# Berkeley-Speech-Group/sylber

Measured on AMD Instinct MI355X. Metric: audio-sec/s encoded (sylber_base, 16 kHz, batched 10 s clips), higher is better.
Workload: dtype bf16

## Files before the change

### include/sylber_hip.h

```cpp
#ifndef SYLBER_HIP_H
#define SYLBER_HIP_H

#include <stdint.h>

#ifdef __cplusplus
extern "C" {
#endif

#define SYLBER_MAX_LAYERS 12
#define SYLBER_HIDDEN 768
#define SYLBER_CONV_DIM 512

typedef struct sylber_ctx* sylber_t;

enum { SYLBER_BF16 = 0, SYLBER_FP32 = 1, SYLBER_FP8 = 2, SYLBER_FP16 = 3, SYLBER_MIXED16 = 4, SYLBER_SPLIT16 = 5 };

typedef struct {
    const float* q_w; const float* q_b;
    const float* k_w; const float* k_b;
    const float* v_w; const float* v_b;
    const float* o_w; const float* o_b;
    const float* ln1_w; const float* ln1_b;
    const float* ff1_w; const float* ff1_b;
    const float* ff2_w; const float* ff2_b;
// ... 78 lines not shown
int sylber_mlp_create(const SylberMlpWeights* w, int device, sylber_mlp_t* out);
void sylber_mlp_destroy(sylber_mlp_t m);
int64_t sylber_condition_workspace_floats(sylber_mlp_t m, int32_t B, int32_t S);
int sylber_condition(sylber_mlp_t m, const float* hidden_dev, const int64_t* seg_dev, const int32_t* nseg_dev, const float* feat_dev,
                     int32_t B, int32_t T, int32_t S, float norm_thr, float* avg_hidden_dev, float* cond_dev, float* workspace_dev,
                     void* stream);

int64_t sylber_condition_units_workspace_floats(sylber_mlp_t m, int32_t B, int32_t S);
int sylber_condition_units(sylber_mlp_t m, const float* c1_dev, int32_t K1, const float* c2_dev, int32_t K2, const int32_t* units_dev,
                           const int32_t* spans_dev, const int32_t* nunits_dev, const int32_t* frames_dev, int32_t B, int32_t T, int32_t S,
                           float* cond_dev, float* workspace_dev, void* stream);
int64_t sylber_condition_packed_workspace_floats(sylber_mlp_t m, int32_t B, int32_t S);
int sylber_condition_packed(sylber_mlp_t m, const float* hidden_dev, const int32_t* offsets_host, const int32_t* frames_host, int32_t B,
                            const int64_t* seg_dev, const int32_t* nseg_dev, const float* feat_dev, int32_t K, int32_t S, float norm_thr,
                            float* avg_hidden_dev, float* cond_dev, float* workspace_dev, void* stream);
int sylber_condition_units_packed(sylber_mlp_t m, const float* c1_dev, int32_t K1, const float* c2_dev, int32_t K2, const int32_t* units_dev,
                                  const int32_t* spans_dev, const int32_t* nunits_dev, const int32_t* frames_host, int32_t B, int32_t S,
                                  float* cond_dev, float* workspace_dev, void* stream);
int sylber_expand_units(const float* feats_dev, const int32_t* durations_dev, int32_t B, int32_t S, int32_t D, int32_t T, float* out_dev,
                        int32_t* workspace_dev, void* stream);

enum { SYLBER_OPT_GEMM_TILE = 1, SYLBER_OPT_ATTN_QUERIES_PER_WAVE = 2, SYLBER_OPT_GEMM_PERSISTENT = 3, SYLBER_OPT_FUSE_OUTPROJ_LN = 4,
       SYLBER_OPT_CONV0_VALU = 5, SYLBER_OPT_RESLN_PREFETCH = 6, SYLBER_OPT_FP8_ATTENTION = 7, SYLBER_OPT_GEMM_TAIL = 8, SYLBER_OPT_SEGMENT = 9, SYLBER_OPT_FP16_AUDIT = 10, SYLBER_OPT_GEMM_H192 = 11, SYLBER_OPT_GEMM_MODEL = 12, SYLBER_OPT_GEMM_MFMA16 = 13,
       SYLBER_OPT_PER_UTTERANCE = 14 };
int sylber_set_option(sylber_t h, int32_t key, int32_t value);
int sylber_get_fp16_audit(sylber_t h, const char** names, uint32_t* saturated, float* max_abs, int32_t cap);

int sylber_condition_features(sylber_mlp_t m, const float* features_dev, int32_t rows, float* cond_dev, float* workspace_dev,
                              void* stream);

int sylber_set_stop_stage(sylber_t h, int32_t stage);
int sylber_set_profiling(sylber_t h, int32_t enable);
int sylber_get_profile(sylber_t h, const char** names, float* ms, int32_t cap);
int sylber_set_graph_mode(sylber_t h, int32_t enable);
int64_t sylber_workspace_bytes(sylber_t h);

#define SYLBER_CFM_DEPTH 8
typedef struct {
    const float *attn_gamma_w, *attn_gamma_b, *attn_beta_w, *attn_beta_b;
    const float *q_gamma, *k_gamma;
    const float *qkv_w, *out_w;
    const float *ff_gamma_w, *ff_gamma_b, *ff_beta_w, *ff_beta_b;
    const float *ff1_w, *ff1_b, *ff2_w, *ff2_b;
} SylberCfmLayer;
typedef struct {
    const float *proj_in_w, *proj_in_b;
    const float *time_freq, *time_w, *time_b;
// ... 41 lines not shown
```

### include/sylber_hip_dev.h

```cpp
#ifndef SYLBER_HIP_DEV_H
#define SYLBER_HIP_DEV_H
#include <stdint.h>
#include "sylber_hip.h"
#ifdef __cplusplus
extern "C" {
#endif
int sylber_debug_gemm_bench(int32_t M, int32_t N, int32_t K, int32_t ldx, int32_t epi, int32_t act, int32_t cfg,
                            int32_t iters, float* ms_out);
int sylber_debug_gemm_pick(int32_t M, int32_t N, int32_t K, int32_t epi, int32_t act, int32_t fmt, int32_t model, int32_t kpat);
int sylber_debug_gemm_trace(int32_t M, int32_t N, int32_t K, int32_t ldx, int32_t epi, int32_t act, unsigned long long* out20,
                            float* ms_out);
int sylber_debug_poison_workspace(sylber_t h, int32_t byte);
int sylber_debug_attention_bench(int32_t B, int32_t T, int32_t precision, int32_t iters, float* ms_out);
#ifdef __cplusplus
}
#endif
#endif
```

### sylber_amd/_lib.py

```python
from __future__ import annotations

import ctypes
import os
from ctypes import POINTER, c_char_p, c_float, c_int, c_int32, c_int64, c_void_p

_HERE = os.path.dirname(os.path.abspath(__file__))
LIB_PATH = os.path.join(_HERE, "libsylber_hip.so")
_DEV_LIB = False
MAX_LAYERS = 12

c_float_p = POINTER(c_float)


class SylberLayerWeights(ctypes.Structure):
    _fields_ = [(n, c_float_p) for n in (
        "q_w", "q_b", "k_w", "k_b", "v_w", "v_b", "o_w", "o_b", "ln1_w", "ln1_b",
        "ff1_w", "ff1_b", "ff2_w", "ff2_b", "ln2_w", "ln2_b")]


class SylberMlpHidden(ctypes.Structure):
    _fields_ = [(n, c_float_p) for n in ("lin_w", "lin_b", "ff1_w", "ff1_b", "ff2_w", "ff2_b", "ln_w", "ln_b")]


class SylberMlpWeights(ctypes.Structure):
# ... 90 lines not shown
    "sylber_packed_layout": (c_int, [POINTER(c_int32), c_int32, POINTER(c_int32), POINTER(c_int32)]),
    "sylber_forward_packed": (c_int, [c_void_p, c_void_p, POINTER(c_int32), c_int32, c_void_p, c_void_p]),
    "sylber_packed_gather": (c_int, [c_void_p, POINTER(c_int32), c_int32, c_void_p, c_void_p]),
    "sylber_segment_packed": (c_int, [c_void_p, c_void_p, POINTER(c_int32), c_int32, c_float, c_float, c_void_p, c_void_p, c_void_p,
                                      c_void_p]),
    "sylber_cfm_packed_layout": (c_int, [POINTER(c_int32), c_int32, POINTER(c_int32)]),
    "sylber_cfm_workspace_bytes_packed": (c_int64, [c_void_p, POINTER(c_int32), c_int32]),
    "sylber_cfm_sample_packed": (c_int, [c_void_p, c_void_p, POINTER(c_int32), c_int32, c_int32, c_void_p, c_float, c_void_p, c_void_p,
                                         c_void_p]),
    "sylber_condition_packed_workspace_floats": (c_int64, [c_void_p, c_int32, c_int32]),
    "sylber_condition_packed": (c_int, [c_void_p, c_void_p, POINTER(c_int32), POINTER(c_int32), c_int32, c_void_p, c_void_p, c_void_p,
                                        c_int32, c_int32, c_float, c_void_p, c_void_p, c_void_p, c_void_p]),
    "sylber_condition_units_packed": (c_int, [c_void_p, c_void_p, c_int32, c_void_p, c_int32, c_void_p, c_void_p, c_void_p,
                                              POINTER(c_int32), c_int32, c_int32, c_void_p, c_void_p, c_void_p]),
    "sylber_op_attention": (c_int, [c_void_p, c_void_p, c_void_p, c_void_p, c_void_p, c_int32, c_int32, c_int32,
                                    c_int32, c_void_p]),
}
DEV_EXPORTS = {
    "sylber_debug_gemm_bench": (c_int, [c_int32] * 8 + [POINTER(c_float)]),
    "sylber_debug_gemm_pick": (c_int, [c_int32] * 8),
    "sylber_debug_gemm_trace": (c_int, [c_int32] * 6 + [POINTER(ctypes.c_uint64), POINTER(c_float)]),
    "sylber_debug_attention_bench": (c_int, [c_int32] * 4 + [POINTER(c_float)]),
    "sylber_debug_poison_workspace": (c_int, [c_void_p, c_int32]),
}
OPT_GEMM_TILE, OPT_ATTN_QUERIES_PER_WAVE, OPT_GEMM_PERSISTENT = 1, 2, 3
OPT_CONV0_VALU = 5
OPT_FP8_ATTENTION, OPT_SEGMENT, OPT_PER_UTTERANCE = 7, 9, 14

_LIB = None


class SylberHipError(RuntimeError):
    pass


def load() -> ctypes.CDLL:
    global _LIB
    if _LIB is None:
        if not os.path.exists(LIB_PATH):
            raise SylberHipError(
                "libsylber_hip.so is not built (%s). Run `python -c 'import __graft_entry__ as g; g.build()'` "
                "or `python sylber_amd/build.py`; there is no CPU fallback on the product path." % LIB_PATH)
        lib = ctypes.CDLL(LIB_PATH)
        for name, (res, args) in list(EXPORTS.items()) + list(DEV_EXPORTS.items()):
            if _DEV_LIB and not hasattr(lib, name):
                continue
            fn = getattr(lib, name)
            fn.restype = res
            fn.argtypes = args
        _LIB = lib
# ... 14 lines not shown
```

### sylber_amd/csrc/api.hip

```cpp
#include <stdio.h>
#include <stdlib.h>
#include <string.h>

#include <string>
#include <vector>

#include "../../include/sylber_hip.h"
#include "../../include/sylber_hip_dev.h"
#include "kernels.h"

static thread_local char g_err[512] = "";
void syl_set_error(const char* what, const char* detail) { snprintf(g_err, sizeof(g_err), "%s: %s", what, detail); }
extern "C" const char* sylber_last_error(void) { return g_err; }

struct DeviceGuard {
    int prev = -1; bool ok = true;
    explicit DeviceGuard(int dev) {
        if (hipGetDevice(&prev) != hipSuccess) prev = -1;
        if (prev != dev) ok = hipSetDevice(dev) == hipSuccess;
    }
    ~DeviceGuard() { int cur = -1; if (prev >= 0 && hipGetDevice(&cur) == hipSuccess && cur != prev) (void)hipSetDevice(prev); }
};
#define GUARD_DEVICE(dev)                                                                             \
    DeviceGuard _dg(dev);                                                                             \
// ... 36 lines not shown
    return 0;
}

struct LayerDev {
    bf16_t *wqkv, *wo, *w1, *w2;
    uint8_t *w1q = nullptr, *w1s = nullptr, *w2q = nullptr, *w2s = nullptr;
    uint8_t *wqkvq = nullptr, *wqkvs = nullptr;
    uint8_t *woq = nullptr, *wos = nullptr;
    float *bqkv, *bo, *b1, *b2, *ln1w, *ln1b, *ln2w, *ln2b;
};

struct ProfEntry { std::string name; hipEvent_t e0, e1; };
struct GraphEntry { int B, Lmax, stop_stage; const void* in; void* out; hipGraphExec_t exec; unsigned long long stamp; };

struct sylber_ctx {
    int device = 0, precision = 0, num_layers = 9;
    int fmt = FMT_BF16;
    int fmt_conv = FMT_BF16;
    char* wbase = nullptr; size_t wbytes = 0;
    char* f8base = nullptr; size_t f8bytes = 0;
    float *conv0_w, *gn_w, *gn_b, *fp_ln_w, *fp_ln_b, *fp_b, *pos_b, *enc_ln_w, *enc_ln_b;
    bf16_t* conv_w[7];
    bf16_t *fp_w, *pos_w;
    LayerDev L[SYLBER_MAX_LAYERS];
    float* conv_w32[7]; float *fp_w32, *pos_w32;
    struct { float *wqkv, *wo, *w1, *w2; } L32[SYLBER_MAX_LAYERS];
    char* ws = nullptr; size_t ws_bytes = 0;
    int ws_B = 0, ws_Lmax = 0;
    float* seg_scratch = nullptr; size_t seg_scratch_floats = 0;
    int stop_stage = 0;
    int opt_gemm_cfg = 0, opt_attn_qw = 0, opt_gemm_persist = 0;
    int opt_fuse_ln = 0;
    int opt_conv0_valu = 0;
    int opt_audit16 = 0;
    unsigned* audit_dev = nullptr;
    int opt_segment = 0;
    int opt_gemm_model = 0;
    int opt_gemm_mfma16 = 0;
    int opt_gemm_h192 = 0;
    int opt_gemm_tail = 0;
    int opt_attn8 = 0;
    int opt_resln_pre = 0;
    int opt_per_utt = 0;
    bool graph_mode = false;
    std::vector<GraphEntry> graphs; unsigned long long graph_clock = 0;
    int profiling = 0;
    std::vector<ProfEntry> prof;
    std::vector<hipEvent_t> ev_pool;
    std::vector<std::string> prof_names; std::vector<float> prof_ms;
};

struct Packer {
    std::vector<char> host;
    size_t add(size_t bytes) { size_t off = (host.size() + 255) & ~(size_t)255; host.resize(off + bytes); return off; }
    size_t add_f32(const float* src, size_t n) { size_t o = add(n * 4); memcpy(host.data() + o, src, n * 4); return o; }
    int fmt = FMT_BF16;
    size_t add_bf16(const float* src, size_t n) {
        if (fmt == FMT_SPLIT) {
            size_t o = add(n * 4);
            bf16_t* d = (bf16_t*)(host.data() + o);
            for (size_t i = 0; i < n; ++i) { d[i] = f2h_host(src[i]); d[n + i] = f2h_host(src[i] - h2f_host(d[i])); }
            return o;
        }
        size_t o = add(n * 2);
        bf16_t* d = (bf16_t*)(host.data() + o);
        if (fmt == FMT_F16) for (size_t i = 0; i < n; ++i) d[i] = f2h_host(src[i]);
// ... 35 lines not shown
    }
    P.fmt = c->fmt;
    size_t o_fplw = P.add_f32(w->fp_ln_w, 512), o_fplb = P.add_f32(w->fp_ln_b, 512);
    size_t o_fpw = f32 ? P.add_f32(w->fp_w, 768 * 512) : P.add_bf16(w->fp_w, 768 * 512), o_fpb = P.add_f32(w->fp_b, 768);
    size_t o_posw;
    {
        std::vector<float> tmp((size_t)16 * 128 * 64 * 56, 0.f);
        for (int g = 0; g < 16; ++g)
            for (int n = 0; n < 48; ++n)
                for (int cc = 0; cc < 48; ++cc)
                    for (int t = 0; t < 128; ++t)
                        tmp[(((size_t)g * 128 + t) * 64 + n) * 56 + cc] = w->pos_w[(((size_t)g * 48 + n) * 48 + cc) * 128 + t];
        if (!f32) o_posw = P.add_bf16(tmp.data(), tmp.size());
        else {
            std::vector<float> t32((size_t)16 * 128 * 64 * 52, 0.f);
            for (int g = 0; g < 16; ++g)
                for (int n = 0; n < 48; ++n)
                    for (int cc = 0; cc < 48; ++cc)
                        for (int t = 0; t < 128; ++t)
                            t32[(((size_t)g * 128 + t) * 64 + n) * 52 + cc] = w->pos_w[(((size_t)g * 48 + n) * 48 + cc) * 128 + t];
            o_posw = P.add_f32(t32.data(), t32.size());
        }
    }
    size_t o_posb = P.add_f32(w->pos_b, 768);
    size_t o_elw = P.add_f32(w->enc_ln_w, 768), o_elb = P.add_f32(w->enc_ln_b, 768);
    struct LOff { size_t wqkv, bqkv, wo, bo, l1w, l1b, w1, b1, w2, b2, l2w, l2b; } lo[SYLBER_MAX_LAYERS];
    for (int l = 0; l < w->num_layers; ++l) {
        const SylberLayerWeights& lw = w->layers[l];
        std::vector<float> qkv((size_t)2304 * 768), bq(2304);
        memcpy(qkv.data(), lw.q_w, 768 * 768 * 4);
        memcpy(qkv.data() + 768 * 768, lw.k_w, 768 * 768 * 4);
        memcpy(qkv.data() + 2 * 768 * 768, lw.v_w, 768 * 768 * 4);
        memcpy(bq.data(), lw.q_b, 768 * 4); memcpy(bq.data() + 768, lw.k_b, 768 * 4); memcpy(bq.data() + 1536, lw.v_b, 768 * 4);
        lo[l].wqkv = f32 ? P.add_f32(qkv.data(), qkv.size()) : P.add_bf16(qkv.data(), qkv.size()); lo[l].bqkv = P.add_f32(bq.data(), 2304);
        lo[l].wo = f32 ? P.add_f32(lw.o_w, 768 * 768) : P.add_bf16(lw.o_w, 768 * 768); lo[l].bo = P.add_f32(lw.o_b, 768);
        lo[l].l1w = P.add_f32(lw.ln1_w, 768); lo[l].l1b = P.add_f32(lw.ln1_b, 768);
        lo[l].w1 = f32 ? P.add_f32(lw.ff1_w, (size_t)3072 * 768) : P.add_bf16(lw.ff1_w, (size_t)3072 * 768); lo[l].b1 = P.add_f32(lw.ff1_b, 3072);
        lo[l].w2 = f32 ? P.add_f32(lw.ff2_w, (size_t)768 * 3072) : P.add_bf16(lw.ff2_w, (size_t)768 * 3072); lo[l].b2 = P.add_f32(lw.ff2_b, 768);
        lo[l].l2w = P.add_f32(lw.ln2_w, 768); lo[l].l2b = P.add_f32(lw.ln2_b, 768);
    }
    c->wbytes = P.host.size();
    if (hipMalloc((void**)&c->wbase, c->wbytes) != hipSuccess) { delete c; syl_set_error("sylber_create", "hipMalloc(weights) failed"); return 1; }
    if (hipMemcpy(c->wbase, P.host.data(), c->wbytes, hipMemcpyHostToDevice) != hipSuccess) {
        hipFree(c->wbase); delete c; syl_set_error("sylber_create", "weight upload failed"); return 1;
    }
    char* b = c->wbase;
    c->conv0_w = (float*)(b + o_conv0); c->gn_w = (float*)(b + o_gnw); c->gn_b = (float*)(b + o_gnb);
    c->conv_w[0] = nullptr;
    for (int i = 1; i < 7; ++i) { c->conv_w[i] = (bf16_t*)(b + o_conv[i]); c->conv_w32[i] = (float*)(b + o_conv[i]); }
    c->fp_w32 = (float*)(b + o_fpw); c->pos_w32 = (float*)(b + o_posw);
    c->fp_ln_w = (float*)(b + o_fplw); c->fp_ln_b = (float*)(b + o_fplb);
    c->fp_w = (bf16_t*)(b + o_fpw); c->fp_b = (float*)(b + o_fpb);
    c->pos_w = (bf16_t*)(b + o_posw); c->pos_b = (float*)(b + o_posb);
    c->enc_ln_w = (float*)(b + o_elw); c->enc_ln_b = (float*)(b + o_elb);
    for (int l = 0; l < w->num_layers; ++l) {
        LayerDev& d = c->L[l];
        d.wqkv = (bf16_t*)(b + lo[l].wqkv); d.bqkv = (float*)(b + lo[l].bqkv);
        d.wo = (bf16_t*)(b + lo[l].wo); d.bo = (float*)(b + lo[l].bo);
        d.ln1w = (float*)(b + lo[l].l1w); d.ln1b = (float*)(b + lo[l].l1b);
        d.w1 = (bf16_t*)(b + lo[l].w1); d.b1 = (float*)(b + lo[l].b1);
        d.w2 = (bf16_t*)(b + lo[l].w2); d.b2 = (float*)(b + lo[l].b2);
        d.ln2w = (float*)(b + lo[l].l2w); d.ln2b = (float*)(b + lo[l].l2b);
        c->L32[l].wqkv = (float*)(b + lo[l].wqkv); c->L32[l].wo = (float*)(b + lo[l].wo);
        c->L32[l].w1 = (float*)(b + lo[l].w1); c->L32[l].w2 = (float*)(b + lo[l].w2);
    }
    if (precision == SYLBER_FP8) {
        const size_t per_layer = (size_t)3072 * 768 + (size_t)3072 * 24 + (size_t)768 * 3072 + (size_t)768 * 96 +
                                 (size_t)2304 * 768 + (size_t)2304 * 24 + (size_t)768 * 768 + (size_t)768 * 24;
        c->f8bytes = per_layer * w->num_layers;
        float* tmp = nullptr;
        if (hipMalloc((void**)&c->f8base, c->f8bytes) != hipSuccess || hipMalloc((void**)&tmp, (size_t)3072 * 768 * 4) != hipSuccess) {
            if (c->f8base) hipFree(c->f8base);
            hipFree(c->wbase); delete c; syl_set_error("sylber_create", "hipMalloc(fp8 weights) failed"); return 1;
        }
        int bad = 0;
        for (int l = 0; l < w->num_layers && !bad; ++l) {
// ... 48 lines not shown
        case SYLBER_OPT_GEMM_TILE: c->opt_gemm_cfg = value < 0 ? 0 : value + 1; break;
        case SYLBER_OPT_ATTN_QUERIES_PER_WAVE: c->opt_attn_qw = value == 32 ? 1 : (value == 64 ? 2 : 0); break;
        case SYLBER_OPT_GEMM_PERSISTENT: c->opt_gemm_persist = value; break;
        case SYLBER_OPT_FUSE_OUTPROJ_LN: c->opt_fuse_ln = value > 0 ? 1 : (value < 0 ? -1 : 0); break;
        case SYLBER_OPT_CONV0_VALU: c->opt_conv0_valu = value > 0 ? (value == 2 ? 2 : 1) : 0; break;
        case SYLBER_OPT_RESLN_PREFETCH: c->opt_resln_pre = value < 0 ? -1 : (value <= 3 ? value : 0); break;
        case SYLBER_OPT_FP8_ATTENTION: c->opt_attn8 = value < 0 ? -1 : (value > 0 ? 1 : 0); break;
        case SYLBER_OPT_FP16_AUDIT: {
            GUARD_DEVICE(c->device);
            c->opt_audit16 = value > 0 ? 1 : 0;
            if (c->opt_audit16) {
                if (!c->audit_dev) HIP_TRY(hipMalloc((void**)&c->audit_dev, AUDIT_STAGES * 2 * sizeof(unsigned)));
                HIP_TRY(hipDeviceSynchronize());
                HIP_TRY(hipMemset(c->audit_dev, 0, AUDIT_STAGES * 2 * sizeof(unsigned)));
            }
            break;
        }
        case SYLBER_OPT_SEGMENT: c->opt_segment = value < 0 ? -1 : 0; break;
        case SYLBER_OPT_GEMM_MODEL: c->opt_gemm_model = value == 5 ? 5 : (value == 2 ? 2 : (value == 6 ? 6 : 0)); break;
        case SYLBER_OPT_GEMM_H192: c->opt_gemm_h192 = value < 0 ? -1 : 0; break;
        case SYLBER_OPT_GEMM_MFMA16: c->opt_gemm_mfma16 = value < 0 ? -1 : 0; break;
        case SYLBER_OPT_GEMM_TAIL: c->opt_gemm_tail = value < 0 ? -1 : (value > 0 ? value + 1 : 0); break;
        case SYLBER_OPT_PER_UTTERANCE: c->opt_per_utt = value == 1 ? 1 : 0; break;
        default: syl_set_error("sylber_set_option", "unknown option key"); return 1;
    }
    if (c->graph_mode) { for (auto& g : c->graphs) if (g.exec) hipGraphExecDestroy(g.exec); c->graphs.clear(); }
    return 0;
}
extern "C" int sylber_set_profiling(sylber_t c, int32_t enable) {
    if (!c) return 1;
    const char* nm[1]; float ms[1];
    sylber_get_profile(c, nm, ms, 0);
    c->prof_names.clear(); c->prof_ms.clear();
    c->profiling = enable;
    return 0;
}
extern "C" int64_t sylber_workspace_bytes(sylber_t c) { return c ? (int64_t)(c->ws_bytes + c->seg_scratch_floats * 4 + c->wbytes + c->f8bytes) : 0; }

struct Plan {
    int B, Lmax, L[7], T, Tp, Tpv, R[7];
    size_t o_bufA, o_bufB, o_ln512, o_xf32, o_xpad, o_pre, o_stats, o_hbf16, o_q, o_k, o_vt, o_ctx, o_ffn, o_part, o_ss, o_valid,
        o_rows, o_pk, total;
    int nchunk;
    bool zero_all = false;
    long lo_bufA = 0, lo_bufB = 0, lo_ln512 = 0, lo_xpad = 0, lo_hbf = 0, lo_qk = 0, lo_vt = 0, lo_ctx = 0, lo_ffn = 0;
};
// ... 241 lines not shown
        bf16_t* t = src; src = dst; dst = t;
        const long tl = src_lo; src_lo = dst_lo; dst_lo = tl;
    }
    bf16_t* feats = src;
    const long feats_lo = src_lo;
    if (c->stop_stage == 1) {
        RUN("copy_out", launch_bf16_to_f32_rows(feats, 512, hidden_dev, B, p.Tp, p.T, 512, s, c->fmt_conv, feats_lo));
        return 0;
    }
    {
        LnArgs a = {};
        a.in = feats; a.in_bf16 = 1; a.ld_in = 512; a.gamma = c->fp_ln_w; a.beta = c->fp_ln_b;
        a.out_bf16 = ln512; a.ld_bf16 = 512; a.M = M; a.D = 512; a.fmt = c->fmt; a.fmt_in = c->fmt_conv;
        a.in_lo = feats_lo; a.out_lo = p.lo_ln512;
        RUN("ln512", launch_layernorm(a, s));
        GemmArgs g = {};
        g.X = ln512; g.ldx = 512; g.W = c->fp_w; g.M = M; g.N = 768; g.K = 512; g.bias = c->fp_b;
        g.out0 = xf32; g.ld0 = 768; g.out1 = xpad; g.Tp = p.Tp; g.T = p.T; g.valid = valid; g.xpad_rows = p.Tp + 128; g.fmt = c->fmt;
        g.x_lo = p.lo_ln512; g.w_lo = (long)768 * 512; g.out_lo = p.lo_xpad;
        RUN("gemm_proj", launch_gemm_bf16(EPI_PROJ, g, s));
        if (pk) RUN("zero_slot_tails", launch_zero_slot_tails(xf32, xpad, pk->slot, pk->frames, pk->nclip, pk->tail_max, s));
        if (aud_e && (audit16(c, AUD_LN512, ln512, M, 512, 512, s) || audit16(c, AUD_XPAD, xpad, (long)B * (p.Tp + 128), 768, 768, s))) return 1;
    }
    if (pk) RUN("posconv", launch_posconv_packed(xpad, c->pos_w, c->pos_b, xf32, pre, pk->nclip, pk->slot_max, pk->slot, pk->frames, s, c->fmt));
    else
    RUN("posconv", launch_posconv(xpad, c->pos_w, c->pos_b, xf32, pre, B, p.Tp, split ? 2 : 1, s, c->fmt, p.lo_xpad, (long)16 * 128 * 64 * 56));
    const bool f8 = c->precision == SYLBER_FP8;
    const long Mp = ((long)M + 255) & ~255L;
    uint8_t* h8 = (uint8_t*)hbf; uint8_t* h8s = h8 + (((size_t)M * 768 + 255) & ~(size_t)255);
    uint8_t* ctx8 = (uint8_t*)ctx; uint8_t* ctx8s = ctx8 + (((size_t)M * 768 + 255) & ~(size_t)255);
    uint8_t* ffn8 = (uint8_t*)ffn; uint8_t* ffn8s = ffn8 + (((size_t)M * 3072 + 255) & ~(size_t)255);
    auto run_ln = [&](const float* gam, const float* bet, bool last, bool to_fp8 = false) -> int {
        LnArgs a = {};
        a.in = pre; a.in_bf16 = 0; a.ld_in = 768; a.gamma = gam; a.beta = bet; a.M = M; a.D = 768; a.fmt = c->fmt; a.fmt_in = c->fmt;
        if (last) { a.out_f32 = hidden_dev; a.ld_f32 = 768; a.Tp = p.Tp; a.T = p.T; }
        else if (to_fp8) { a.out_fp8 = h8; a.ld_fp8 = 768; a.out_scale = h8s; a.scale_rows = Mp; a.out_stats = stats; }
        else { a.out_bf16 = hbf; a.ld_bf16 = 768; a.out_stats = stats; a.out_lo = p.lo_hbf; }
        if (launch_layernorm(a, s)) return 1;
        if (aud_e && !last && !to_fp8) return audit16(c, AUD_LN, hbf, M, 768, 768, s);
        return 0;
    };
    RUN("layernorm", run_ln(c->enc_ln_w, c->enc_ln_b, c->stop_stage == 2, f8));
    if (c->stop_stage == 2) return 0;
    const float* res_g = c->enc_ln_w; const float* res_b = c->enc_ln_b;
    for (int l = 0; l < c->num_layers; ++l) {
        const LayerDev& d = c->L[l];
        const bool last = (l == c->num_layers - 1) || (c->stop_stage == 3 + l);
        bool fused_ln1 = false;
        uint8_t* q8 = (uint8_t*)q; uint8_t* k8 = (uint8_t*)k; uint8_t* v8 = (uint8_t*)vt;
// ... 593 lines not shown
    if (qb.alloc(n * 2) || kb.alloc(n * 2 + 64 * 64 * 2) || vb.alloc((size_t)B * 768 * Tpv * 2) || cb.alloc(n * 2)) { syl_set_error("sylber_op_attention", "alloc"); return 1; }
    HIP_TRY(hipMemsetAsync(qb.p, 0, n * 2, s)); HIP_TRY(hipMemsetAsync(kb.p, 0, n * 2 + 64 * 64 * 2, s));
    HIP_TRY(hipMemsetAsync(vb.p, 0, (size_t)B * 768 * Tpv * 2, s)); HIP_TRY(hipMemsetAsync(cb.p, 0, n * 2, s));
    hipLaunchKernelGGL(pack_qkv_kernel, dim3(T, B), dim3(256), 0, s, q_dev, k_dev, v_dev, (bf16_t*)qb.p, (bf16_t*)kb.p, (bf16_t*)vb.p, T, Tp, Tpv);
    if (launch_attention((bf16_t*)qb.p, (bf16_t*)kb.p, (bf16_t*)vb.p, valid_dev, (bf16_t*)cb.p, B, T, Tp, Tpv, qw, s)) return 1;
    if (launch_bf16_to_f32_rows((bf16_t*)cb.p, 768, o_dev, B, Tp, T, 768, s)) return 1;
    HIP_TRY(hipStreamSynchronize(s));
    return 0;
}


__global__ void fill_random_bf16(bf16_t* p, size_t n, unsigned seed);
extern "C" int sylber_debug_poison_workspace(sylber_t c, int32_t byte) {
    if (!c) { syl_set_error("sylber_debug_poison_workspace", "null handle"); return 1; }
    GUARD_DEVICE(c->device);
    HIP_TRY(hipDeviceSynchronize());
    if (c->ws) HIP_TRY(hipMemset(c->ws, byte & 0xff, c->ws_bytes));
    if (c->seg_scratch) HIP_TRY(hipMemset(c->seg_scratch, byte & 0xff, c->seg_scratch_floats * 4));
    c->ws_B = 0; c->ws_Lmax = 0;
    if (c->graph_mode) { for (auto& g : c->graphs) if (g.exec) hipGraphExecDestroy(g.exec); c->graphs.clear(); }
    return 0;
}

extern "C" int sylber_debug_attention_bench(int32_t B, int32_t T, int32_t precision, int32_t iters, float* ms_out) {
    const int Tp = (T + 31) & ~31, Tpv = (Tp + 63) & ~63;
    const size_t n = (size_t)B * Tp * 768;
    TmpBuf qin;
    if (qin.alloc((size_t)B * T * 768 * 4 * 3)) { syl_set_error("sylber_debug_attention_bench", "alloc"); return 1; }
    float* q = (float*)qin.p; float* k = q + (size_t)B * T * 768; float* v = k + (size_t)B * T * 768;
    const bool zero_data = iters < 0;
    if (zero_data) { iters = -iters; HIP_TRY(hipMemset(qin.p, 0, (size_t)B * T * 768 * 4 * 3)); }
    else
    {
        TmpBuf tmp;
        if (tmp.alloc((size_t)B * T * 768 * 3 * 2)) { syl_set_error("sylber_debug_attention_bench", "alloc"); return 1; }
        hipLaunchKernelGGL(fill_random_bf16, dim3(2048), dim3(256), 0, 0, (bf16_t*)tmp.p, (size_t)B * T * 768 * 3, 7u);
        if (launch_bf16_to_f32_rows((bf16_t*)tmp.p, 768, q, 3 * B, T, T, 768, 0)) return 1;
        HIP_TRY(hipDeviceSynchronize());
    }
    hipEvent_t e0, e1;
    hipEventCreate(&e0); hipEventCreate(&e1);
    int rc = 0;
    if (precision == SYLBER_FP8) {
        AttnF8Bufs f;
        if (f.alloc(B, Tp, Tpv) || f.clear(B, Tp, Tpv, 0)) { syl_set_error("sylber_debug_attention_bench", "alloc"); return 1; }
        hipLaunchKernelGGL(pack_qk_f8_kernel, dim3(T, B), dim3(256), 0, 0, q, k, (uint8_t*)f.q8.p, (uint8_t*)f.qs.p, (uint8_t*)f.k8.p, (uint8_t*)f.ks.p, T, Tp);
// ... 183 lines not shown
```

### sylber_amd/csrc/kernels.h

```cpp
#pragma once
#include "common.h"

enum GemmAct { ACT_NONE = 0, ACT_GELU_FAST = 1, ACT_GELU_ERF = 2, ACT_GELU_ERF7 = 3 };
enum GemmEpi {
    EPI_BF16 = 0,
    EPI_F32 = 1,
    EPI_F32_RES = 2,
    EPI_QK = 3,
    EPI_PROJ = 4,
    EPI_MXFP8 = 7,
    EPI_QK8 = 8,
    EPI_F32_RESLN = 6,
};

struct GemmArgs {
    const bf16_t* X; long ldx;
    const bf16_t* W;
    int M, N, K;
    int M_store;
    const float* bias;
    int act;
    void* out0; long ld0;
    void* out1; void* out2;
    const float* res; long ldres;
// ... 47 lines not shown
enum GemmActF32 { ACTF_NONE = 0, ACTF_GELU_ERF = 1, ACTF_RELU = 2 };
struct GemmArgsF32 {
    const float* X; long ldx;
    const float* W;
    int M, N, K;
    const float* bias; int act;
    float* out0; long ld0;
    const float* res; long ldres;
    int Tp, T; const int* valid;
    float* xpad; int xpad_rows;
    int tiled;
};
int launch_gemm_f32(const GemmArgsF32& a, hipStream_t s);

int launch_conv0_stats(const float* wav, int B, int Lmax, int L0, double* partials, int nchunk, hipStream_t s, const int* rows = nullptr,
                       const int* slot = nullptr);
int launch_conv0_finalize(const double* partials, int nchunk, const float* w0, const float* gn_w, const float* gn_b,
                          int B, int L0, float* scale_shift, hipStream_t s, const int* rows = nullptr);
int launch_conv0_gn_gelu(const float* wav, int B, int Lmax, int L0, int R0, const float* w0,
                         const float* scale_shift, void* out, int out_f32, hipStream_t s, int fmt = 0, long out_lo = 0, int valu16 = 0);
int launch_conv0_packed(const float* wav, int B, int total_samples, int slot_max, const int* rows, const int* slot, const float* w0,
                        const float* scale_shift, bf16_t* out, int fmt, hipStream_t s);
int launch_zero_slot_tails(float* x, bf16_t* xpad, const int* slot, const int* frames, int B, int tail_max, hipStream_t s);
int launch_posconv_packed(const bf16_t* xpad, const bf16_t* wpk, const float* bias, const float* x_f32, float* out, int B, int slot_max,
                          const int* slot, const int* frames, hipStream_t s, int fmt);
int launch_attention_packed(const bf16_t* q, const bf16_t* k, const bf16_t* vt, const int* pk, int nclip, int total_qb, bf16_t* ctx,
                            int Ptot, hipStream_t s, int fmt);

struct LnArgs {
    const void* in; int in_bf16; long ld_in;
    int fmt;
    int fmt_in;
    const float* res; long ld_res;
    const float* gamma; const float* beta;
    float* out_f32; long ld_f32;
    bf16_t* out_bf16; long ld_bf16;
    uint8_t* out_fp8; long ld_fp8;
    uint8_t* out_scale; long scale_rows;
    float* out_stats;
    int M, D;
    int Tp, T;
    long in_lo, out_lo;
};
int launch_layernorm(const LnArgs& a, hipStream_t s);

int launch_attention(const bf16_t* q, const bf16_t* k, const bf16_t* vt, const int* valid, bf16_t* ctx, int B, int T,
                     int Tp, int Tpv, int qw, hipStream_t s, int fmt = 0, long lo_qk = 0, long lo_vt = 0, long lo_ctx = 0);
int launch_attention_f8(const uint8_t* q8, const uint8_t* qs, const uint8_t* k8, const uint8_t* ks, const uint8_t* v8, const uint8_t* vs,
                        const int* valid, void* ctx, uint8_t* ctx_scale, long scale_rows, int B, int T, int Tp, int Tpv, hipStream_t s);
int launch_attention_f8out(const bf16_t* q, const bf16_t* k, const bf16_t* vt, const int* valid, uint8_t* ctx8, uint8_t* ctx_scale,
                           long scale_rows, int B, int T, int Tp, int Tpv, int qw, hipStream_t s);
int launch_attention_f32(const float* q, const float* k, const float* v, const int* valid, float* ctx, int B, int T,
                         int Tp, hipStream_t s);

int launch_posconv(const bf16_t* xpad, const bf16_t* wpk, const float* bias, const float* x_f32, float* out, int B,
                   int Tp, int act, hipStream_t s, int fmt = 0, long x_lo = 0, long w_lo = 0);
int launch_posconv_f32(const float* xpad, const float* w, const float* bias, const float* x_f32, float* out, int B,
                       int Tp, hipStream_t s);

int launch_segment(const float* hidden, int B, int T, int D, float norm_thr, float merge_thr, int64_t* seg, int* nseg,
                   float* feat, float* scratch, hipStream_t s, int mode = 0, const int* frames = nullptr, const int* row0 = nullptr);
size_t segment_scratch_floats(int B, int T, int D);

int launch_upload_ints(int* dst, const int32_t* vals_host, int n, int add, hipStream_t s);
int launch_f32_to_bf16(const float* in, bf16_t* out, size_t n, hipStream_t s);
int launch_f32_to_split16(const float* in, bf16_t* out, long lo_off, size_t n, hipStream_t s);
int launch_bf16_to_f32_rows(const bf16_t* in, long ld_in, float* out, int B, int Tp, int T, int D, hipStream_t s, int fmt = 0, long in_lo = 0);
```

### sylber_amd/csrc/posconv.hip

```cpp
#include "kernels.h"

#define PC_BM 256
#define PC_XROW 112
#define PC_XWIN (384 * PC_XROW)
#define PC_SLAB (64 * 112)
#define PC_TAPS_PER_STEP 2
#define PC_STEP (PC_TAPS_PER_STEP * PC_SLAB)
#define PC_LDS (PC_XWIN + 2 * PC_STEP)

typedef __attribute__((address_space(3))) void* lds_vptr;
typedef const __attribute__((address_space(1))) void* glb_vptr;
__device__ __forceinline__ void glds16p(__amdgpu_buffer_rsrc_t rs, int voff, int soff, void* l) {
    __builtin_amdgcn_raw_ptr_buffer_load_lds(rs, (lds_vptr)l, 16, voff, soff, 0, 0);
}

template <int ACT, int FMT>
__global__ __launch_bounds__(512, 4) void posconv_bf16_kernel(const bf16_t* __restrict__ xpad, const bf16_t* __restrict__ wpk,
                                                              const float* __restrict__ bias, const float* __restrict__ x_f32,
                                                              float* __restrict__ out, int Tp, long x_lo, long w_lo,
                                                              const int* __restrict__ slot, const int* __restrict__ frames) {
    extern __shared__ __attribute__((aligned(256))) char smem[];
    char* xwin = smem;
    char* wring = smem + PC_XWIN;
    const int tid = threadIdx.x, wave = tid >> 6, lane = tid & 63;
// ... 71 lines not shown
    }
    const int t = t0 + wave * 32 + ql;
    if (t < Tpb) {
        const size_t m = slot ? (size_t)s0 + t : (size_t)b * Tp + t;
#pragma unroll
        for (int nf = 0; nf < 2; ++nf)
#pragma unroll
            for (int gg = 0; gg < 4; ++gg) {
                const int nl = 32 * nf + 8 * gg + 4 * h;
                if (nl >= SYL_POSC) continue;
                const int n = g * SYL_POSC + nl;
                const float4 bb = *(const float4*)(bias + n);
                const float4 rr = *(const float4*)(x_f32 + m * SYL_HIDDEN + n);
                float v0 = acc[nf][4 * gg + 0] + bb.x, v1 = acc[nf][4 * gg + 1] + bb.y;
                float v2 = acc[nf][4 * gg + 2] + bb.z, v3 = acc[nf][4 * gg + 3] + bb.w;
                if constexpr (ACT == 2 && FMT == FMT_SPLIT) { v0 = gelu_erf7(v0); v1 = gelu_erf7(v1); v2 = gelu_erf7(v2); v3 = gelu_erf7(v3); }
                else if constexpr (ACT == 2) { v0 = gelu_erf(v0); v1 = gelu_erf(v1); v2 = gelu_erf(v2); v3 = gelu_erf(v3); }
                else { v0 = gelu_fast(v0); v1 = gelu_fast(v1); v2 = gelu_fast(v2); v3 = gelu_fast(v3); }
                *(float4*)(out + m * SYL_HIDDEN + n) = make_float4(rr.x + v0, rr.y + v1, rr.z + v2, rr.w + v3);
            }
    }
}

static int posconv_attrs() {
    static PerDeviceOnce attr_once;
    if (attr_once.need()) {
        HIP_TRY(hipFuncSetAttribute((const void*)posconv_bf16_kernel<1, FMT_BF16>, hipFuncAttributeMaxDynamicSharedMemorySize, PC_LDS));
        HIP_TRY(hipFuncSetAttribute((const void*)posconv_bf16_kernel<2, FMT_BF16>, hipFuncAttributeMaxDynamicSharedMemorySize, PC_LDS));
        HIP_TRY(hipFuncSetAttribute((const void*)posconv_bf16_kernel<1, FMT_F16>, hipFuncAttributeMaxDynamicSharedMemorySize, PC_LDS));
        HIP_TRY(hipFuncSetAttribute((const void*)posconv_bf16_kernel<2, FMT_SPLIT>, hipFuncAttributeMaxDynamicSharedMemorySize, PC_LDS));
    }
    return 0;
}

int launch_posconv(const bf16_t* xpad, const bf16_t* wpk, const float* bias, const float* x_f32, float* out, int B, int Tp,
                   int act, hipStream_t s, int fmt, long x_lo, long w_lo) {
    dim3 grid((Tp + PC_BM - 1) / PC_BM, SYL_POSG, B);
    if (posconv_attrs()) return 1;
    if (fmt == FMT_SPLIT) {
        hipLaunchKernelGGL((posconv_bf16_kernel<2, FMT_SPLIT>), grid, dim3(512), PC_LDS, s, xpad, wpk, bias, x_f32, out, Tp, x_lo, w_lo, nullptr, nullptr);
        HIP_TRY(hipGetLastError());
        return 0;
    }
    if (fmt == FMT_F16 && act == 2) { syl_set_error("launch_posconv", "the erf GELU (act 2) has no fp16 instantiation"); return 1; }
    if (fmt == FMT_F16) hipLaunchKernelGGL((posconv_bf16_kernel<1, FMT_F16>), grid, dim3(512), PC_LDS, s, xpad, wpk, bias, x_f32, out, Tp, 0L, 0L, nullptr, nullptr);
    else if (act == 2) hipLaunchKernelGGL((posconv_bf16_kernel<2, FMT_BF16>), grid, dim3(512), PC_LDS, s, xpad, wpk, bias, x_f32, out, Tp, 0L, 0L, nullptr, nullptr);
    else hipLaunchKernelGGL((posconv_bf16_kernel<1, FMT_BF16>), grid, dim3(512), PC_LDS, s, xpad, wpk, bias, x_f32, out, Tp, 0L, 0L, nullptr, nullptr);
    HIP_TRY(hipGetLastError());
    return 0;
}

int launch_posconv_packed(const bf16_t* xpad, const bf16_t* wpk, const float* bias, const float* x_f32, float* out, int B, int slot_max,
                          const int* slot, const int* frames, hipStream_t s, int fmt) {
    if (fmt != FMT_BF16 && fmt != FMT_F16) { syl_set_error("launch_posconv_packed", "bf16 / fp16 only"); return 1; }
    if (posconv_attrs()) return 1;
    dim3 grid((slot_max + PC_BM - 1) / PC_BM, SYL_POSG, B);
    if (fmt == FMT_F16) hipLaunchKernelGGL((posconv_bf16_kernel<1, FMT_F16>), grid, dim3(512), PC_LDS, s, xpad, wpk, bias, x_f32, out, 0, 0L, 0L, slot, frames);
    else hipLaunchKernelGGL((posconv_bf16_kernel<1, FMT_BF16>), grid, dim3(512), PC_LDS, s, xpad, wpk, bias, x_f32, out, 0, 0L, 0L, slot, frames);
    HIP_TRY(hipGetLastError());
    return 0;
}
```

Measured before the change: 67150.

## Add 16x16x32 MFMA positional-conv kernel with repacked per-tap weights

Adds a new positional convolution kernel that uses 16x16x32 bf16/f16 MFMA instructions over an LDS-resident input window. Weights are repacked at load time into per-tap 48x48 slabs and streamed through a double-buffered LDS ring. It is enabled by default for 16-bit single-plane formats and can be turned off through a new option. The aim is higher matrix-core efficiency for the grouped conv. The cost is extra weight memory and a new code path that could be numerically or layout sensitive.

```diff
diff --git a/include/sylber_hip.h b/include/sylber_hip.h
--- a/include/sylber_hip.h
+++ b/include/sylber_hip.h
@@ -124,7 +124,7 @@
 
 enum { SYLBER_OPT_GEMM_TILE = 1, SYLBER_OPT_ATTN_QUERIES_PER_WAVE = 2, SYLBER_OPT_GEMM_PERSISTENT = 3, SYLBER_OPT_FUSE_OUTPROJ_LN = 4,
        SYLBER_OPT_CONV0_VALU = 5, SYLBER_OPT_RESLN_PREFETCH = 6, SYLBER_OPT_FP8_ATTENTION = 7, SYLBER_OPT_GEMM_TAIL = 8, SYLBER_OPT_SEGMENT = 9, SYLBER_OPT_FP16_AUDIT = 10, SYLBER_OPT_GEMM_H192 = 11, SYLBER_OPT_GEMM_MODEL = 12, SYLBER_OPT_GEMM_MFMA16 = 13,
-       SYLBER_OPT_PER_UTTERANCE = 14 };
+       SYLBER_OPT_PER_UTTERANCE = 14, SYLBER_OPT_POSCONV_MFMA16 = 15 };
 int sylber_set_option(sylber_t h, int32_t key, int32_t value);
 int sylber_get_fp16_audit(sylber_t h, const char** names, uint32_t* saturated, float* max_abs, int32_t cap);
 
diff --git a/include/sylber_hip_dev.h b/include/sylber_hip_dev.h
--- a/include/sylber_hip_dev.h
+++ b/include/sylber_hip_dev.h
@@ -11,6 +11,8 @@
 int sylber_debug_gemm_trace(int32_t M, int32_t N, int32_t K, int32_t ldx, int32_t epi, int32_t act, unsigned long long* out20,
                             float* ms_out);
 int sylber_debug_poison_workspace(sylber_t h, int32_t byte);
+int sylber_debug_posconv(sylber_t h, const void* xpad_dev, const float* x_dev, float* out_dev, int32_t B, int32_t Tp, const int32_t* slot_dev,
+                         const int32_t* frames_dev, int32_t slot_max);
 int sylber_debug_attention_bench(int32_t B, int32_t T, int32_t precision, int32_t iters, float* ms_out);
 #ifdef __cplusplus
 }
diff --git a/sylber_amd/_lib.py b/sylber_amd/_lib.py
--- a/sylber_amd/_lib.py
+++ b/sylber_amd/_lib.py
@@ -136,10 +136,12 @@
     "sylber_debug_gemm_trace": (c_int, [c_int32] * 6 + [POINTER(ctypes.c_uint64), POINTER(c_float)]),
     "sylber_debug_attention_bench": (c_int, [c_int32] * 4 + [POINTER(c_float)]),
     "sylber_debug_poison_workspace": (c_int, [c_void_p, c_int32]),
+    "sylber_debug_posconv": (c_int, [c_void_p, c_void_p, c_void_p, c_void_p, c_int32, c_int32, c_void_p, c_void_p, c_int32]),
 }
 OPT_GEMM_TILE, OPT_ATTN_QUERIES_PER_WAVE, OPT_GEMM_PERSISTENT = 1, 2, 3
 OPT_CONV0_VALU = 5
 OPT_FP8_ATTENTION, OPT_SEGMENT, OPT_PER_UTTERANCE = 7, 9, 14
+OPT_POSCONV_MFMA16 = 15
 
 _LIB = None
 
diff --git a/sylber_amd/csrc/api.hip b/sylber_amd/csrc/api.hip
--- a/sylber_amd/csrc/api.hip
+++ b/sylber_amd/csrc/api.hip
@@ -82,6 +82,7 @@
     float *conv0_w, *gn_w, *gn_b, *fp_ln_w, *fp_ln_b, *fp_b, *pos_b, *enc_ln_w, *enc_ln_b;
     bf16_t* conv_w[7];
     bf16_t *fp_w, *pos_w;
+    bf16_t* pos_w16 = nullptr;
     LayerDev L[SYLBER_MAX_LAYERS];
     float* conv_w32[7]; float *fp_w32, *pos_w32;
     struct { float *wqkv, *wo, *w1, *w2; } L32[SYLBER_MAX_LAYERS];
@@ -102,6 +103,7 @@
     int opt_attn8 = 0;
     int opt_resln_pre = 0;
     int opt_per_utt = 0;
+    int opt_posconv16 = 0;
     bool graph_mode = false;
     std::vector<GraphEntry> graphs; unsigned long long graph_clock = 0;
     int profiling = 0;
@@ -183,6 +185,17 @@
             o_posw = P.add_f32(t32.data(), t32.size());
         }
     }
+    size_t o_posw16 = 0;
+    const bool posw16 = !f32 && c->fmt != FMT_SPLIT;
+    if (posw16) {
+        std::vector<float> tmp((size_t)16 * 128 * 48 * 48);
+        for (int g = 0; g < 16; ++g)
+            for (int n = 0; n < 48; ++n)
+                for (int cc = 0; cc < 48; ++cc)
+                    for (int t = 0; t < 128; ++t)
+                        tmp[(((size_t)g * 128 + t) * 48 + n) * 48 + cc] = w->pos_w[(((size_t)g * 48 + n) * 48 + cc) * 128 + t];
+        o_posw16 = P.add_bf16(tmp.data(), tmp.size());
+    }
     size_t o_posb = P.add_f32(w->pos_b, 768);
     size_t o_elw = P.add_f32(w->enc_ln_w, 768), o_elb = P.add_f32(w->enc_ln_b, 768);
     struct LOff { size_t wqkv, bqkv, wo, bo, l1w, l1b, w1, b1, w2, b2, l2w, l2b; } lo[SYLBER_MAX_LAYERS];
@@ -213,6 +226,7 @@
     c->fp_ln_w = (float*)(b + o_fplw); c->fp_ln_b = (float*)(b + o_fplb);
     c->fp_w = (bf16_t*)(b + o_fpw); c->fp_b = (float*)(b + o_fpb);
     c->pos_w = (bf16_t*)(b + o_posw); c->pos_b = (float*)(b + o_posb);
+    if (posw16) c->pos_w16 = (bf16_t*)(b + o_posw16);
     c->enc_ln_w = (float*)(b + o_elw); c->enc_ln_b = (float*)(b + o_elb);
     for (int l = 0; l < w->num_layers; ++l) {
         LayerDev& d = c->L[l];
@@ -307,6 +321,7 @@
         case SYLBER_OPT_GEMM_MFMA16: c->opt_gemm_mfma16 = value < 0 ? -1 : 0; break;
         case SYLBER_OPT_GEMM_TAIL: c->opt_gemm_tail = value < 0 ? -1 : (value > 0 ? value + 1 : 0); break;
         case SYLBER_OPT_PER_UTTERANCE: c->opt_per_utt = value == 1 ? 1 : 0; break;
+        case SYLBER_OPT_POSCONV_MFMA16: c->opt_posconv16 = value < 0 ? -1 : 0; break;
         default: syl_set_error("sylber_set_option", "unknown option key"); return 1;
     }
     if (c->graph_mode) { for (auto& g : c->graphs) if (g.exec) hipGraphExecDestroy(g.exec); c->graphs.clear(); }
@@ -594,9 +609,10 @@
         if (pk) RUN("zero_slot_tails", launch_zero_slot_tails(xf32, xpad, pk->slot, pk->frames, pk->nclip, pk->tail_max, s));
         if (aud_e && (audit16(c, AUD_LN512, ln512, M, 512, 512, s) || audit16(c, AUD_XPAD, xpad, (long)B * (p.Tp + 128), 768, 768, s))) return 1;
     }
-    if (pk) RUN("posconv", launch_posconv_packed(xpad, c->pos_w, c->pos_b, xf32, pre, pk->nclip, pk->slot_max, pk->slot, pk->frames, s, c->fmt));
+    const bf16_t* pos_w16 = c->opt_posconv16 < 0 ? nullptr : c->pos_w16;
+    if (pk) RUN("posconv", launch_posconv_packed(xpad, c->pos_w, pos_w16, c->pos_b, xf32, pre, pk->nclip, pk->slot_max, pk->slot, pk->frames, s, c->fmt));
     else
-    RUN("posconv", launch_posconv(xpad, c->pos_w, c->pos_b, xf32, pre, B, p.Tp, split ? 2 : 1, s, c->fmt, p.lo_xpad, (long)16 * 128 * 64 * 56));
+    RUN("posconv", launch_posconv(xpad, c->pos_w, pos_w16, c->pos_b, xf32, pre, B, p.Tp, split ? 2 : 1, s, c->fmt, p.lo_xpad, (long)16 * 128 * 64 * 56));
     const bool f8 = c->precision == SYLBER_FP8;
     const long Mp = ((long)M + 255) & ~255L;
     uint8_t* h8 = (uint8_t*)hbf; uint8_t* h8s = h8 + (((size_t)M * 768 + 255) & ~(size_t)255);
@@ -1236,6 +1252,19 @@
     return 0;
 }
 
+extern "C" int sylber_debug_posconv(sylber_t c, const void* xpad_dev, const float* x_dev, float* out_dev, int32_t B, int32_t Tp,
+                                    const int32_t* slot_dev, const int32_t* frames_dev, int32_t slot_max) {
+    if (!c || !xpad_dev || !x_dev || !out_dev || B < 1) { syl_set_error("sylber_debug_posconv", "null argument or B < 1"); return 1; }
+    if (c->precision == SYLBER_FP32 || c->fmt == FMT_SPLIT) { syl_set_error("sylber_debug_posconv", "16-bit single-plane handles only"); return 1; }
+    GUARD_DEVICE(c->device);
+    const bf16_t* w16 = c->opt_posconv16 < 0 ? nullptr : c->pos_w16;
+    const int rc = slot_dev ? launch_posconv_packed((const bf16_t*)xpad_dev, c->pos_w, w16, c->pos_b, x_dev, out_dev, B, slot_max, slot_dev, frames_dev, 0, c->fmt)
+                            : launch_posconv((const bf16_t*)xpad_dev, c->pos_w, w16, c->pos_b, x_dev, out_dev, B, Tp, 1, 0, c->fmt);
+    if (rc) return 1;
+    HIP_TRY(hipDeviceSynchronize());
+    return 0;
+}
+
 extern "C" int sylber_debug_attention_bench(int32_t B, int32_t T, int32_t precision, int32_t iters, float* ms_out) {
     const int Tp = (T + 31) & ~31, Tpv = (Tp + 63) & ~63;
     const size_t n = (size_t)B * Tp * 768;
diff --git a/sylber_amd/csrc/kernels.h b/sylber_amd/csrc/kernels.h
--- a/sylber_amd/csrc/kernels.h
+++ b/sylber_amd/csrc/kernels.h
@@ -93,8 +93,8 @@
 int launch_conv0_packed(const float* wav, int B, int total_samples, int slot_max, const int* rows, const int* slot, const float* w0,
                         const float* scale_shift, bf16_t* out, int fmt, hipStream_t s);
 int launch_zero_slot_tails(float* x, bf16_t* xpad, const int* slot, const int* frames, int B, int tail_max, hipStream_t s);
-int launch_posconv_packed(const bf16_t* xpad, const bf16_t* wpk, const float* bias, const float* x_f32, float* out, int B, int slot_max,
-                          const int* slot, const int* frames, hipStream_t s, int fmt);
+int launch_posconv_packed(const bf16_t* xpad, const bf16_t* wpk, const bf16_t* w16, const float* bias, const float* x_f32, float* out, int B,
+                          int slot_max, const int* slot, const int* frames, hipStream_t s, int fmt);
 int launch_attention_packed(const bf16_t* q, const bf16_t* k, const bf16_t* vt, const int* pk, int nclip, int total_qb, bf16_t* ctx,
                             int Ptot, hipStream_t s, int fmt);
 
@@ -124,7 +124,7 @@
 int launch_attention_f32(const float* q, const float* k, const float* v, const int* valid, float* ctx, int B, int T,
                          int Tp, hipStream_t s);
 
-int launch_posconv(const bf16_t* xpad, const bf16_t* wpk, const float* bias, const float* x_f32, float* out, int B,
+int launch_posconv(const bf16_t* xpad, const bf16_t* wpk, const bf16_t* w16, const float* bias, const float* x_f32, float* out, int B,
                    int Tp, int act, hipStream_t s, int fmt = 0, long x_lo = 0, long w_lo = 0);
 int launch_posconv_f32(const float* xpad, const float* w, const float* bias, const float* x_f32, float* out, int B,
                        int Tp, hipStream_t s);
diff --git a/sylber_amd/csrc/posconv.hip b/sylber_amd/csrc/posconv.hip
--- a/sylber_amd/csrc/posconv.hip
+++ b/sylber_amd/csrc/posconv.hip
@@ -117,6 +117,116 @@
     }
 }
 
+#define P16_XROW 96
+#define P16_XWIN (384 * P16_XROW)
+#define P16_SLAB (48 * 96)
+#define P16_STEP (2 * P16_SLAB)
+#define P16_LDS (P16_XWIN + 2 * P16_STEP)
+
+template <int FMT> struct PcMF16 {
+    static __device__ __forceinline__ f32x4_t mfma(bf16x8_t a, bf16x8_t b, f32x4_t c) { return __builtin_amdgcn_mfma_f32_16x16x32_bf16(a, b, c, 0, 0, 0); }
+};
+template <> struct PcMF16<FMT_F16> {
+    static __device__ __forceinline__ f32x4_t mfma(bf16x8_t a, bf16x8_t b, f32x4_t c) {
+        return __builtin_amdgcn_mfma_f32_16x16x32_f16(__builtin_bit_cast(f16x8_t, a), __builtin_bit_cast(f16x8_t, b), c, 0, 0, 0);
+    }
+};
+
+template <int ACT, int FMT>
+__global__ __launch_bounds__(512, 2) void posconv16_kernel(const bf16_t* __restrict__ xpad, const bf16_t* __restrict__ wpk,
+                                                           const float* __restrict__ bias, const float* __restrict__ x_f32,
+                                                           float* __restrict__ out, int Tp,
+                                                           const int* __restrict__ slot, const int* __restrict__ frames) {
+    extern __shared__ __attribute__((aligned(256))) char smem[];
+    char* xwin = smem;
+    char* wring = smem + P16_XWIN;
+    const int tid = threadIdx.x, wave = tid >> 6, lane = tid & 63;
+    const int r16 = lane & 15, q = lane >> 4;
+    const int t0 = blockIdx.x * PC_BM, g = blockIdx.y, b = blockIdx.z;
+    const int rows_per_b = Tp + 128;
+    int s0 = 0, Tb = 0, Tpb = Tp;
+    if (slot) {
+        s0 = slot[b]; Tb = frames[b]; Tpb = slot[b + 1] - s0;
+        if (t0 >= Tpb) return;
+    }
+    {
+        const bf16_t* xb = xpad + (slot ? (size_t)s0 : (size_t)b * rows_per_b) * SYL_HIDDEN + g * SYL_POSC;
+#pragma unroll
+        for (int i = 0; i < 5; ++i) {
+            const int idx = tid + 512 * i;
+            if (idx < 384 * 6) {
+                const int r = idx / 6, ch = idx - r * 6;
+                uint4 v;
+                if (slot) {
+                    const int f = t0 + r - 64;
+                    v = (f >= 0 && f < Tb) ? *(const uint4*)(xb + (size_t)(f + 64) * SYL_HIDDEN + ch * 8) : make_uint4(0u, 0u, 0u, 0u);
+                } else {
+                    int row = t0 + r; row = row < rows_per_b ? row : rows_per_b - 1;
+                    v = *(const uint4*)(xb + (size_t)row * SYL_HIDDEN + ch * 8);
+                }
+                *(uint4*)(xwin + idx * 16) = v;
+            }
+        }
+    }
+    const char* wg_base = (const char*)wpk + (size_t)g * SYL_POSK * P16_SLAB;
+    const __amdgpu_buffer_rsrc_t rwg = __builtin_amdgcn_make_buffer_rsrc((void*)wg_base, 0, (int)0xffffffffu, 0x00020000);
+    auto stage = [&](int step, int buf) {
+        char* dst = wring + buf * P16_STEP;
+        glds16p(rwg, wave * 1024 + lane * 16, step * P16_STEP, dst + wave * 1024);
+        if (wave == 0) glds16p(rwg, 8 * 1024 + lane * 16, step * P16_STEP, dst + 8 * 1024);
+    };
+    const int xfrag = (wave * 32 + r16) * P16_XROW + q * 16;
+    int wfrag[3];
+#pragma unroll
+    for (int kc = 0; kc < 3; ++kc) {
+        const int k0 = 32 * kc + 8 * q, tt = k0 >= 48 ? 1 : 0, c0 = k0 - 48 * tt;
+        wfrag[kc] = tt * P16_SLAB + r16 * 96 + c0 * 2;
+    }
+    f32x4_t acc[2][3];
+#pragma unroll
+    for (int i = 0; i < 2; ++i)
+#pragma unroll
+        for (int j = 0; j < 3; ++j) acc[i][j] = f32x4_t{0.f, 0.f, 0.f, 0.f};
+
+    const int nsteps = SYL_POSK / 2;
+    stage(0, 0);
+    for (int st = 0; st < nsteps; ++st) {
+        asm volatile("s_waitcnt vmcnt(0)" ::: "memory");
+        __syncthreads();
+        if (st + 1 < nsteps) stage(st + 1, (st + 1) & 1);
+        const char* wb = wring + (st & 1) * P16_STEP;
+        const char* xs = xwin + xfrag + st * 2 * P16_XROW;
+#pragma unroll
+        for (int kc = 0; kc < 3; ++kc) {
+            bf16x8_t xf[2], wf[3];
+#pragma unroll
+            for (int ff = 0; ff < 2; ++ff) xf[ff] = *(const bf16x8_t*)(xs + ff * 16 * P16_XROW + kc * 64);
+#pragma unroll
+            for (int nf = 0; nf < 3; ++nf) wf[nf] = *(const bf16x8_t*)(wb + wfrag[kc] + nf * 16 * 96);
+#pragma unroll
+            for (int ff = 0; ff < 2; ++ff)
+#pragma unroll
+                for (int nf = 0; nf < 3; ++nf) acc[ff][nf] = PcMF16<FMT>::mfma(wf[nf], xf[ff], acc[ff][nf]);
+        }
+    }
+#pragma unroll
+    for (int ff = 0; ff < 2; ++ff) {
+        const int t = t0 + wave * 32 + ff * 16 + r16;
+        if (t >= Tpb) continue;
+        const size_t m = slot ? (size_t)s0 + t : (size_t)b * Tp + t;
+#pragma unroll
+        for (int nf = 0; nf < 3; ++nf) {
+            const int n = g * SYL_POSC + 16 * nf + 4 * q;
+            const float4 bb = *(const float4*)(bias + n);
+            const float4 rr = *(const float4*)(x_f32 + m * SYL_HIDDEN + n);
+            float v0 = acc[ff][nf][0] + bb.x, v1 = acc[ff][nf][1] + bb.y, v2 = acc[ff][nf][2] + bb.z, v3 = acc[ff][nf][3] + bb.w;
+            if constexpr (ACT == 2) { v0 = gelu_erf(v0); v1 = gelu_erf(v1); v2 = gelu_erf(v2); v3 = gelu_erf(v3); }
+            else { v0 = gelu_fast(v0); v1 = gelu_fast(v1); v2 = gelu_fast(v2); v3 = gelu_fast(v3); }
+            *(float4*)(out + m * SYL_HIDDEN + n) = make_float4(rr.x + v0, rr.y + v1, rr.z + v2, rr.w + v3);
+        }
+    }
+}
+
 static int posconv_attrs() {
     static PerDeviceOnce attr_once;
     if (attr_once.need()) {
@@ -124,11 +234,14 @@
         HIP_TRY(hipFuncSetAttribute((const void*)posconv_bf16_kernel<2, FMT_BF16>, hipFuncAttributeMaxDynamicSharedMemorySize, PC_LDS));
         HIP_TRY(hipFuncSetAttribute((const void*)posconv_bf16_kernel<1, FMT_F16>, hipFuncAttributeMaxDynamicSharedMemorySize, PC_LDS));
         HIP_TRY(hipFuncSetAttribute((const void*)posconv_bf16_kernel<2, FMT_SPLIT>, hipFuncAttributeMaxDynamicSharedMemorySize, PC_LDS));
+        HIP_TRY(hipFuncSetAttribute((const void*)posconv16_kernel<1, FMT_BF16>, hipFuncAttributeMaxDynamicSharedMemorySize, P16_LDS));
+        HIP_TRY(hipFuncSetAttribute((const void*)posconv16_kernel<2, FMT_BF16>, hipFuncAttributeMaxDynamicSharedMemorySize, P16_LDS));
+        HIP_TRY(hipFuncSetAttribute((const void*)posconv16_kernel<1, FMT_F16>, hipFuncAttributeMaxDynamicSharedMemorySize, P16_LDS));
     }
     return 0;
 }
 
-int launch_posconv(const bf16_t* xpad, const bf16_t* wpk, const float* bias, const float* x_f32, float* out, int B, int Tp,
+int launch_posconv(const bf16_t* xpad, const bf16_t* wpk, const bf16_t* w16, const float* bias, const float* x_f32, float* out, int B, int Tp,
                    int act, hipStream_t s, int fmt, long x_lo, long w_lo) {
     dim3 grid((Tp + PC_BM - 1) / PC_BM, SYL_POSG, B);
     if (posconv_attrs()) return 1;
@@ -138,19 +251,28 @@
         return 0;
     }
     if (fmt == FMT_F16 && act == 2) { syl_set_error("launch_posconv", "the erf GELU (act 2) has no fp16 instantiation"); return 1; }
-    if (fmt == FMT_F16) hipLaunchKernelGGL((posconv_bf16_kernel<1, FMT_F16>), grid, dim3(512), PC_LDS, s, xpad, wpk, bias, x_f32, out, Tp, 0L, 0L, nullptr, nullptr);
+    if (w16) {
+        if (fmt == FMT_F16) hipLaunchKernelGGL((posconv16_kernel<1, FMT_F16>), grid, dim3(512), P16_LDS, s, xpad, w16, bias, x_f32, out, Tp, nullptr, nullptr);
+        else if (act == 2) hipLaunchKernelGGL((posconv16_kernel<2, FMT_BF16>), grid, dim3(512), P16_LDS, s, xpad, w16, bias, x_f32, out, Tp, nullptr, nullptr);
+        else hipLaunchKernelGGL((posconv16_kernel<1, FMT_BF16>), grid, dim3(512), P16_LDS, s, xpad, w16, bias, x_f32, out, Tp, nullptr, nullptr);
+    }
+    else if (fmt == FMT_F16) hipLaunchKernelGGL((posconv_bf16_kernel<1, FMT_F16>), grid, dim3(512), PC_LDS, s, xpad, wpk, bias, x_f32, out, Tp, 0L, 0L, nullptr, nullptr);
     else if (act == 2) hipLaunchKernelGGL((posconv_bf16_kernel<2, FMT_BF16>), grid, dim3(512), PC_LDS, s, xpad, wpk, bias, x_f32, out, Tp, 0L, 0L, nullptr, nullptr);
     else hipLaunchKernelGGL((posconv_bf16_kernel<1, FMT_BF16>), grid, dim3(512), PC_LDS, s, xpad, wpk, bias, x_f32, out, Tp, 0L, 0L, nullptr, nullptr);
     HIP_TRY(hipGetLastError());
     return 0;
 }
 
-int launch_posconv_packed(const bf16_t* xpad, const bf16_t* wpk, const float* bias, const float* x_f32, float* out, int B, int slot_max,
-                          const int* slot, const int* frames, hipStream_t s, int fmt) {
+int launch_posconv_packed(const bf16_t* xpad, const bf16_t* wpk, const bf16_t* w16, const float* bias, const float* x_f32, float* out, int B,
+                          int slot_max, const int* slot, const int* frames, hipStream_t s, int fmt) {
     if (fmt != FMT_BF16 && fmt != FMT_F16) { syl_set_error("launch_posconv_packed", "bf16 / fp16 only"); return 1; }
     if (posconv_attrs()) return 1;
     dim3 grid((slot_max + PC_BM - 1) / PC_BM, SYL_POSG, B);
-    if (fmt == FMT_F16) hipLaunchKernelGGL((posconv_bf16_kernel<1, FMT_F16>), grid, dim3(512), PC_LDS, s, xpad, wpk, bias, x_f32, out, 0, 0L, 0L, slot, frames);
+    if (w16) {
+        if (fmt == FMT_F16) hipLaunchKernelGGL((posconv16_kernel<1, FMT_F16>), grid, dim3(512), P16_LDS, s, xpad, w16, bias, x_f32, out, 0, slot, frames);
+        else hipLaunchKernelGGL((posconv16_kernel<1, FMT_BF16>), grid, dim3(512), P16_LDS, s, xpad, w16, bias, x_f32, out, 0, slot, frames);
+    }
+    else if (fmt == FMT_F16) hipLaunchKernelGGL((posconv_bf16_kernel<1, FMT_F16>), grid, dim3(512), PC_LDS, s, xpad, wpk, bias, x_f32, out, 0, 0L, 0L, slot, frames);
     else hipLaunchKernelGGL((posconv_bf16_kernel<1, FMT_BF16>), grid, dim3(512), PC_LDS, s, xpad, wpk, bias, x_f32, out, 0, 0L, 0L, slot, frames);
     HIP_TRY(hipGetLastError());
     return 0;
```

After: 67620 (median of 6 runs). About the same (+0.7%).
